# ChicyChen/LOCO-Edit

Hardware: AMD Instinct MI355X
Metric: edit-directions/sec (top-5 PMP-Jacobian SVD @256^2) + vT cos-sim vs ref (higher is better)
Workload: dtype bf16x3 (split-bf16 MFMA operands, fp32 accumulate + fp32 storage); 1 GPU; CelebA-HQ DDPM 256x256 top-5 local basis (l_eye-sized mask, L=2400), t=0.6T, 12 power iterations, one GPU; multi_gpu_form=single, probes_total=5, probes_per_gpu=5, kept=5, n_iter=12, mask_L=2400, weights=synthetic seed 0, streams=2

## Files before the change

### include/loco_hip_diag.h

```cpp
#ifndef LOCO_HIP_DIAG_H
#define LOCO_HIP_DIAG_H
#include "loco_hip.h"
#ifdef __cplusplus
extern "C" {
#endif

int  loco_bench_conv(loco_ctx* ctx, int32_t cin, int32_t cout, int32_t H, int32_t W, int32_t B, int32_t mode,
                     int32_t taps, int32_t tile, int32_t iters, float* ms_avg, void* stream);

typedef struct loco_conv_desc {
    int32_t struct_size;
    int32_t Cin, Cout, Hin, Win, B, taps;
    int32_t stride, upsample, zins, mode, cpg;
    int32_t transposed, accumulate, in_arena, pad;
    int32_t Cin2, cot_cpg;
    float   res_scale;
    int32_t st_cpg;
    const float *weight, *bias;
    const float *in, *bias2, *res;
    const float *prim, *sc, *sh, *mr, *gamma, *tst, *tc;
    const float *in2, *w2, *bias2nd;
    const float *cot_d, *cot_prim, *cot_sc, *cot_sh, *cot_mr, *cot_tc;
    float* out;
    const float *st_prim, *st_mr;
    float* st_out;
    int32_t pool2;
    int32_t st_kind, st_keep;
    float   st_eps;
    int32_t st_keep_cap;
    const float *st_gamma, *st_beta, *st_ss_scale, *st_ss_shift;
    const float *st_sc, *st_sh;
    float *st_o_mr, *st_o_sc, *st_o_sh;
    float *st_o_tst, *st_o_tc;
    float *st_keep_out;
} loco_conv_desc;
int  loco_debug_conv(loco_ctx* ctx, const loco_conv_desc* desc, char* plan, int64_t cap, void* stream);

typedef struct loco_attn_desc {
    int32_t struct_size;
    int32_t kind, pass;
    int32_t T, NH, CH, B;
    int32_t Lt, L, pair, no_workspace;
    const float *q, *k, *v;
    const float *kt, *vt;
    float *P, *o;
    const float *dq, *dk, *dv;
    float* out;
    const float* go;
    float *gq, *gk, *gv;
} loco_attn_desc;
int  loco_debug_attn(loco_ctx* ctx, const loco_attn_desc* desc, char* route, int64_t cap, void* stream);

typedef struct loco_norm_desc {
    int32_t struct_size;
    int32_t op, kind, act, B, C, HW, G, C1, ntA, ntB, accumulate;
    float   eps, base_scale;
    int64_t x_bs, d_bs, base_bs, out_bs, pbs_c, pbs_g, o_bs, t_bs;
// ... 12 lines not shown
```

### loco-edit_amd/csrc/conv.hip

```cpp
#include "kernels.h"

namespace loco {

typedef float f32x16 __attribute__((ext_vector_type(16)));

constexpr int BK = 8;

template <int MODE>
__device__ __forceinline__ float prologue(float d, float x, float sc, float sh, float gamma, float mean,
                                          float rstd, float m1, float m2, int act) {
    if constexpr (MODE == CM_NONE) {
        return d;
    } else if constexpr (MODE == CM_GN_SILU) {
        return act_fwd(fmaf(sc, d, sh), act);
    } else if constexpr (MODE == CM_GN) {
        return fmaf(sc, d, sh);
    } else {
        float xh = (x - mean) * rstd;
        float ds = act_der(fmaf(sc, x, sh), act);
        if constexpr (MODE == CM_TAN_SILU) {
            return ds * sc * (d - m1 - xh * m2);
        } else {
            return rstd * (gamma * ds * d - m1 - xh * m2);
        }
// ... 283 lines not shown
        const int co = (int)(rem / out_plane);
        f32x4_r v = {0.f, 0.f, 0.f, 0.f};
        const float* pp = a.partial + i;
        int s = 0;
        for (; s + 4 <= a.nsplit; s += 4) {
            const f32x4_r p0 = *reinterpret_cast<const f32x4_r*>(pp + (long)s * total);
            const f32x4_r p1 = *reinterpret_cast<const f32x4_r*>(pp + (long)(s + 1) * total);
            const f32x4_r p2 = *reinterpret_cast<const f32x4_r*>(pp + (long)(s + 2) * total);
            const f32x4_r p3 = *reinterpret_cast<const f32x4_r*>(pp + (long)(s + 3) * total);
            v += (p0 + p1) + (p2 + p3);
        }
        for (; s < a.nsplit; ++s) v += *reinterpret_cast<const f32x4_r*>(pp + (long)s * total);
        float add = 0.f;
        if (a.bias) add += a.bias[co];
        if (a.bias2) add += a.bias2[(long)b * a.bias2_bs + co];
        v += add;
        if (a.res) v += a.res_scale * *reinterpret_cast<const f32x4_r*>(a.res + (long)b * a.res_bs + rem);
        float* o = a.out + (long)b * a.out_bs + rem;
        if (a.accumulate) v += *reinterpret_cast<const f32x4_r*>(o);
        *reinterpret_cast<f32x4_r*>(o) = v;
    }
}

void launch_conv_splitk_reduce(const ConvArgs& a, hipStream_t st) {
    if (a.nsplit > 1) {
        long total = (long)a.B * a.Cout * a.Hout * a.Wout;
        const bool vec = ((a.Hout * a.Wout) % 4) == 0 && (a.out_bs % 4) == 0 && (a.res_bs % 4) == 0 &&
                         (reinterpret_cast<uintptr_t>(a.out) % 16) == 0 && (reinterpret_cast<uintptr_t>(a.res) % 16) == 0;
        if (vec) {
            int blocks = (int)((total / 4 + 255) / 256);
            if (blocks > 2048) blocks = 2048;
            hipLaunchKernelGGL(conv_splitk_reduce4, dim3(blocks), dim3(256), 0, st, a, total);
            return;
        }
        int blocks = (int)((total + 255) / 256);
        if (blocks > 2048) blocks = 2048;
        hipLaunchKernelGGL(conv_splitk_reduce, dim3(blocks), dim3(256), 0, st, a, total);
    }
}

}
```

### loco-edit_amd/csrc/conv_bf16.hip

```cpp
#include "kernels.h"
#include <cstdio>
#include <cstdlib>

namespace loco {

enum : int { PR_BF16X3 = 0, PR_F16 = 1 };
template <int PR, int TAPS, int MODE> void launch_tile_b(const ConvArgs& a, hipStream_t st);
template <int PR, int MODE> void launch_kcat_b(const ConvArgs& a, hipStream_t st);
template <int PR, int MODE> void launch_pair_b(const ConvArgs& a, hipStream_t st);
void launch_conv_gemm(const ConvArgs& a, hipStream_t st);
template <int PR> void launch_poly_b(const ConvArgs& a, hipStream_t st);
template <int PR> void launch_poly_in_b(const ConvArgs& a, hipStream_t st);

template <int PR>
static void launch_lowp(const ConvArgs& a, int taps, hipStream_t st) {
#ifdef LOCO_DIAG
    if (a.cot_d && (taps != 1 || a.gemm || a.nsplit > 1 || a.Cin2 > 0 || (a.Cout % conv_bf16_tile_couts(a)) != 0 || a.st_kind == ST_TAN || a.st_kind == ST_COT)) {
        fprintf(stderr, "loco: ConvArgs::cot_d on a launch whose epilogue has no norm-cotangent term (taps %d, gemm %d, nsplit %d, Cout %d, st_kind %d)\n",
                taps, a.gemm, a.nsplit, a.Cout, a.st_kind);
        abort();
    }
#endif
    if constexpr (PR == PR_BF16X3) {
        if (taps == 1 && a.gemm) { launch_conv_gemm(a, st); return; }
    }
    if (taps == 9 && a.poly == 2) { launch_poly_in_b<PR>(a, st); return; }
    if (taps == 9 && a.poly) { launch_poly_b<PR>(a, st); return; }
    if (taps == 9 && a.Cin2 > 0) {
        if (a.mode == CM_GN_SILU) launch_kcat_b<PR, CM_GN_SILU>(a, st);
        else if (a.mode == CM_GN_GELU) launch_kcat_b<PR, CM_GN_GELU>(a, st);
        else launch_kcat_b<PR, CM_TAN_SILU>(a, st);
        return;
    }
    if constexpr (PR == PR_BF16X3) {
        if (taps == 9 && a.pair) {
            switch (a.mode) {
                case CM_NONE: launch_pair_b<PR, CM_NONE>(a, st); break;
                case CM_GN_SILU: launch_pair_b<PR, CM_GN_SILU>(a, st); break;
                case CM_TAN_SILU: launch_pair_b<PR, CM_TAN_SILU>(a, st); break;
                default: launch_pair_b<PR, CM_COT_SILU>(a, st); break;
            }
            return;
        }
    }
    if (taps == 9) {
        switch (a.mode) {
            case CM_NONE: launch_tile_b<PR, 9, CM_NONE>(a, st); break;
            case CM_GN_SILU: launch_tile_b<PR, 9, CM_GN_SILU>(a, st); break;
            case CM_GN_GELU: launch_tile_b<PR, 9, CM_GN_GELU>(a, st); break;
            case CM_TAN_SILU: launch_tile_b<PR, 9, CM_TAN_SILU>(a, st); break;
            case CM_COT_SILU: launch_tile_b<PR, 9, CM_COT_SILU>(a, st); break;
            default: launch_tile_b<PR, 9, CM_GN>(a, st); break;
        }
    } else {
// ... 11 lines not shown
```

### loco-edit_amd/csrc/conv_bf16_inst_f.hip

```cpp
#include "conv_bf16_kernel.h"

namespace loco {
template void launch_kcat_b<PR_BF16X3, CM_GN_SILU>(const ConvArgs&, hipStream_t);
template void launch_kcat_b<PR_BF16X3, CM_TAN_SILU>(const ConvArgs&, hipStream_t);
template void launch_kcat_b<PR_BF16X3, CM_GN_GELU>(const ConvArgs&, hipStream_t);
}
```

### loco-edit_amd/csrc/conv_bf16_inst_f_f16.hip

```cpp
#include "conv_bf16_kernel.h"

namespace loco {
template void launch_kcat_b<PR_F16, CM_GN_SILU>(const ConvArgs&, hipStream_t);
template void launch_kcat_b<PR_F16, CM_TAN_SILU>(const ConvArgs&, hipStream_t);
template void launch_kcat_b<PR_F16, CM_GN_GELU>(const ConvArgs&, hipStream_t);
}
```

### loco-edit_amd/csrc/conv_bf16_kernel.h

```cpp
#pragma once
#include "kernels.h"
#include <cstdlib>
#include <type_traits>

namespace loco {


typedef float f32x16 __attribute__((ext_vector_type(16)));
typedef float f32x4 __attribute__((ext_vector_type(4)));
typedef f32x4 f32x4_u __attribute__((aligned(4)));
typedef float f32x2 __attribute__((ext_vector_type(2)));
typedef f32x2 f32x2_u __attribute__((aligned(4)));
typedef __bf16 bf16x8 __attribute__((ext_vector_type(8)));
typedef _Float16 f16x8 __attribute__((ext_vector_type(8)));
typedef short s16x8 __attribute__((ext_vector_type(8)));

enum : int { PR_BF16X3 = 0, PR_F16 = 1 };

constexpr int BKC = 16;
constexpr bool LIVE_MASK = true;
constexpr bool EARLY_W = true;
constexpr int NDUMMY = 8;

__device__ __forceinline__ float sigmoidf2_(float y) { return __builtin_amdgcn_rcpf(1.0f + __expf(-y)); }
// ... 1304 lines not shown
            (void)hipFuncSetAttribute(reinterpret_cast<const void*>(kern), hipFuncAttributeMaxDynamicSharedMemorySize,
                                      160 * 1024);
        }
    }
    hipLaunchKernelGGL(kern, grid, dim3(WM * WN * 64), lds, st, a);
}

template <int PR, int TAPS, int WM, int WN, int TM, int TN, int MODE>
static void launch_one_b(const ConvArgs& a, hipStream_t st) {
    const bool general = a.stride != 1 || a.upsample || a.zins || (a.Cin % BKC) != 0 || !a.in_padded;
    if constexpr (MODE == CM_NONE) {
        if (a.stride == 2) launch_one_b2<PR, TAPS, WM, WN, TM, TN, MODE, 2>(a, st);
        else if (TAPS == 9 && !general) launch_one_b2<PR, TAPS, WM, WN, TM, TN, MODE, 0>(a, st);
        else launch_one_b2<PR, TAPS, WM, WN, TM, TN, MODE, 1>(a, st);
        return;
    }
    if constexpr (MODE == CM_GN_SILU || MODE == CM_TAN_SILU || MODE == CM_GN_GELU) {
        if (general) { launch_one_b2<PR, TAPS, WM, WN, TM, TN, MODE, 1>(a, st); return; }
    }
    launch_one_b2<PR, TAPS, WM, WN, TM, TN, MODE, 0>(a, st);
}


template <int PR, int MODE>
void launch_kcat_b(const ConvArgs& a, hipStream_t st) {
    constexpr int WM = 2, WN = 4, TM = 2, TN = 2, MT = 128, NT = 256;
    const int TW = a.Wout < 32 ? a.Wout : 32, TH = NT / TW;
    size_t lds = (size_t)3 * 3 * MT * rec_bytes<PR>() + 2 * ((size_t)(TW + 2) * (TH + 2) + NDUMMY) * halo_pitch<PR>();
    dim3 grid(((a.Hout * a.Wout) / NT) * ((a.Cout + MT - 1) / MT) * a.B * a.nsplit);
    void (*kern)(ConvArgs);
    if constexpr (PR == PR_F16) kern = &conv_kcat_f16<WM, WN, TM, TN, MODE>;
    else kern = &conv_kcat_bf16x3<WM, WN, TM, TN, MODE>;
    static DeviceOnce once;
    if (first_on_device(once))
        (void)hipFuncSetAttribute(reinterpret_cast<const void*>(kern), hipFuncAttributeMaxDynamicSharedMemorySize, 160 * 1024);
    hipLaunchKernelGGL(kern, grid, dim3(WM * WN * 64), lds, st, a);
}

template <int PR>
void launch_poly_b(const ConvArgs& a, hipStream_t st) {
    ConvArgs v = a;
    v.Cout = 4 * a.Cout; v.Hout = a.Hin; v.Wout = a.Win;
    v.upsample = 0; v.zins = 0; v.stride = 1; v.pad = 1; v.nsplit = 1;
    launch_one_b2<PR, 4, 2, 4, 2, 2, CM_NONE, 0>(v, st);
}

template <int PR>
void launch_poly_in_b(const ConvArgs& a, hipStream_t st) {
    ConvArgs v = a;
    v.Cin = 4 * a.Cin; v.Hin = a.Hin / 2; v.Win = a.Win / 2;
    v.upsample = 0; v.zins = 0; v.stride = 1; v.pad = 1; v.nsplit = 1;
// ... 19 lines not shown
```

### loco-edit_amd/csrc/conv_plan.hip

```cpp
#include "kernels.h"
#include <cstdio>
#include <cstdlib>

namespace loco {

constexpr int BKC = 16;
constexpr int BKF = 8;

static const int kMT[6] = {128, 128, 32, 64, 128, 128}, kNT[6] = {128, 64, 128, 64, 256, 256};

static int env_int(const char* name, int dflt) {
    const char* e = getenv(name);
    return e ? atoi(e) : dflt;
}
static int pick_tile(int Cout, int HW) {
    if (HW >= 128) return Cout > 32 ? 0 : 2;
    return Cout > 64 ? 1 : 3;
}

static int conv_pick_nsplit(int Cin, int Cout, int Hout, int Wout, int B) {
    const int t = pick_tile(Cout, Hout * Wout);
    long blocks = (long)((Hout * Wout) / kNT[t]) * ((Cout + kMT[t] - 1) / kMT[t]) * B;
    int nchunks = (Cin + BKF - 1) / BKF;
    if (blocks >= 384 || nchunks < 8) return 1;
// ... 50 lines not shown
static int conv_bf16_pick_nsplit(int Cin, int Cout, int Hout, int Wout, int B, int chip_share, int taps, int lanes) {
    const int HW = Hout * Wout;
    int t = conv_bf16_pick_tile(Cout, HW, B, -1);
    if (t == 4) t = 5;
    if (taps == 1 && t == 5 && B >= 2 && HW <= kTile0MaxHW) t = 0;
    long blocks = (long)(HW / kNT[t]) * ((Cout + kMT[t] - 1) / kMT[t]) * B;
    int nchunks = (Cin + BKC - 1) / BKC;
    int target = chip_share > 1 ? 256 / chip_share : (lanes == 2 ? 240 : 256);
    if (target < 32) target = 32;
    if (blocks >= target / 2 || nchunks < 8) return 1;
    int want = (int)(target / blocks);
    int maxs = nchunks / 4;
    if (want > maxs) want = maxs;
    if (want > 32) want = 32;
    return want < 1 ? 1 : want;
}

static bool conv_lowp_can_kcat(const ConvArgs& a) {
    static const bool on = env_int("LOCO_KCAT", 1) != 0;
    return on && a.Cin2 > 0 && a.nsplit == 1 && bf16_tile_of(a) == 5 && a.stride == 1 && !a.upsample && !a.zins && a.pad == 1 &&
           (a.Cin % BKC) == 0 && (a.Cin2 % BKC) == 0 && a.in_padded &&
           (a.mode == CM_GN_SILU || a.mode == CM_GN_GELU || a.mode == CM_TAN_SILU);
}
static bool conv_lowp_can_fuse_stats(const ConvArgs& a) {
    return a.nsplit <= 1 && !a.gemm && (a.Cout % conv_bf16_tile_couts(a)) == 0;
}

static bool conv_pair_ok(const ConvArgs& a) {
    static const bool on = env_int("LOCO_CONV_PAIR", 1) != 0;
    if (!on || a.poly || a.Hout * a.Wout < 16384 || a.taps != 9 || a.Cin2 > 0 || a.nsplit != 1 || a.stride != 1 || a.upsample || a.zins ||
        a.pad != 1 || !a.in_padded || (a.Cin % (2 * BKC)) != 0 || (a.Cout % 128) != 0 || (a.Wout % 32) != 0 || (a.Hout % 8) != 0)
        return false;
    if (!(a.mode == CM_NONE || a.mode == CM_GN_SILU || a.mode == CM_TAN_SILU || a.mode == CM_COT_SILU)) return false;
    return a.tile == 5;
}

static ConvArgs conv_shift_batch(const ConvArgs& a, int nb) {
    ConvArgs t = a;
    t.B = a.B - nb;
    t.in += (long)nb * a.in_bs; t.out += (long)nb * a.out_bs;
    if (t.prim) t.prim += (long)nb * a.prim_bs;
    if (t.bias2) t.bias2 += (long)nb * a.bias2_bs;
    if (t.res) t.res += (long)nb * a.res_bs;
    if (t.sc) { t.sc += (long)nb * a.scsh_bs; t.sh += (long)nb * a.scsh_bs; }
    if (t.mr) t.mr += (long)nb * a.mr_bs;
    if (t.tst) t.tst += (long)nb * a.tst_bs;
// ... 94 lines not shown
    ConvLaunch l;
    l.args = x;
    l.s0 = s0;
    l.args.tile = tile_for(x, e.prec, -1);
    l.stats = stats_route(e, q, want, l.args, s0, B, keep_ntile);
    if (l.stats == SR_EPI || l.stats == SR_KEEP) l.ntile = (x.Hout * x.Wout) / conv_bf16_tile_pixels(l.args);
    conv_plan_tile_pair(l.args, e.prec, -1);
    return l;
}

ConvPlan plan_conv(const ConvEnv& e, const ConvArgs& a0, int taps, const StatAsk* q, const ConvArgs* sc) {
    ConvPlan p;
    ConvArgs a = a0;
    a.taps = taps;
    a.gemm = 0;
    a.poly = 0;
    if (a.pool2) {
        if (conv_poly_in_ok(e, a, taps)) a.poly = 2;
        else {
            p.pool_after = true; p.pool_out = a.out; p.pool_out_bs = a.out_bs; p.pool_acc = a.accumulate;
            a.out = a.pool_tmp; a.out_bs = a.pool_tmp_bs; a.Hout = a.Hin; a.Wout = a.Win; a.accumulate = 0; a.pool2 = 0;
        }
    }
    if (sc) {
        ConvArgs t = a;
        t.nsplit = e.prec >= 1 ? conv_bf16_pick_nsplit(a.Cin, a.Cout, a.Hout, a.Wout, a.B, e.chip_share, 9, e.lanes) : 2;
        t.in2 = sc->in; t.in2_bs = sc->in_bs; t.Cin2 = sc->Cin;
        const long per_probe = (long)((a.Hout * a.Wout) / 256) * ((a.Cout + 127) / 128);
        if (e.prec >= 1 && taps == 9 && !short_tail(per_probe, a.B) && !a.bias2 && conv_lowp_can_kcat(t)) {
            a.in2 = sc->in; a.in2_bs = sc->in_bs; a.Cin2 = sc->Cin; a.in2_padded = sc->in_padded;
            a.wb2 = e.prec == 2 ? sc->wh : sc->wb;
            a.bias2 = sc->bias; a.bias2_bs = 0;
            a.res = nullptr;
        } else {
            p.sc_first = true;
            a.res = sc->out; a.res_bs = sc->out_bs;
        }
    }
    if (e.prec == 2) a.wb = a.wh;
    a.no_deep = e.deep1 ? 0 : 1;
    a.nsplit = e.prec >= 1 ? conv_bf16_pick_nsplit(a.Cin, a.Cout, a.Hout, a.Wout, a.B, e.chip_share, taps, e.lanes)
                           : conv_pick_nsplit(a.Cin, a.Cout, a.Hout, a.Wout, a.B);
    if (a.cot_d) {
        ConvArgs t = a;
        t.tile = bf16_tile_of(t);
        const long per_probe = (long)((a.Hout * a.Wout) / conv_bf16_tile_pixels(t)) * ((a.Cout + 127) / 128);
        p.cot = e.prec >= 1 && taps == 1 && a.nsplit == 1 && !short_tail(per_probe, a.B) && conv_lowp_can_fuse_stats(t);
        if (!p.cot) { a.cot_d = nullptr; a.cot_d_bs = 0; a.cot_sx = nullptr; a.cot_tc = nullptr; a.cot_tc_bs = 0; }
    }
    while (a.nsplit > 1 && (size_t)a.nsplit * a.B * a.Cout * a.Hout * a.Wout > e.partial_floats) a.nsplit >>= 1;
    if (a.nsplit < 1) a.nsplit = 1;
    a.partial = e.partial;
    a.partial_floats = e.partial_floats;
    if (!a.poly && conv_poly_ok(e, a, taps)) a.poly = 1;
    if (a.poly == 1) { a.nsplit = 1; a.wb = e.prec == 2 ? a.wph : a.wpb; }
    if (a.poly == 2) { a.nsplit = 1; a.wb = e.prec == 2 ? a.wqh : a.wqb; }
    conv_plan_family(a, e.prec);
    a.tile = tile_for(a, e.prec, -1);
    int split = 1;
    const int tail = e.prec >= 1 && a.nsplit == 1 && a.B >= 2 && !a.gemm && !a.poly ? tail_split(a, e.partial_floats, &split) : 0;
    const bool want = q && q->kind != ST_NONE && e.prec >= 1 && e.fuse_stats;
    if (!tail) {
        p.l[0] = plan_launch(e, q, want, a, 0, a.B, &p.keep_ntile);
        return p;
    }
    const bool per_part = want && q->norm && (q->kind == ST_FWD || (e.fuse_lin && (a.Hout * a.Wout) % 4 == 0));
    p.stats_all = !per_part && q && q->kind != ST_NONE && q->norm;
    const StatAsk* ql = per_part ? q : nullptr;
    const int nb = a.B - tail;
    ConvArgs m = a, t = conv_shift_batch(a, nb);
    m.B = nb;
    t.nsplit = split;
    p.nl = 2;
    p.l[0] = plan_launch(e, ql, want, m, 0, a.B, &p.keep_ntile);
// ... 23 lines not shown

void polyphase_fold_in(int nin, int nout, const float* w, long so, long si, long st, float* out, int noutP) {
    for (int p = 0; p < 2; ++p)
        for (int q = 0; q < 2; ++q)
            for (int i = 0; i < nin; ++i)
                for (int ty = 0; ty < 2; ++ty)
                    for (int tx = 0; tx < 2; ++tx) {
                        const int m = 2 * ty + 1 - p, n = 2 * tx + 1 - q;
                        for (int o = 0; o < nout; ++o) {
                            double acc = 0.0;
                            for (int a = 0; a < 2; ++a)
                                for (int b = 0; b < 2; ++b) {
                                    const int ky = m - a, kx = n - b;
                                    if (ky >= 0 && ky < 3 && kx >= 0 && kx < 3) acc += (double)w[o * so + i * si + (3 * ky + kx) * st];
                                }
                            out[((((long)(2 * p + q) * nin + i) * 4) + 2 * ty + tx) * noutP + o] = (float)acc;
                        }
                    }
}

const char* conv_variant_name(const ConvArgs& a, int taps, int prec) {
    static const char* tiles[6] = {"2,2,2,2", "4,1,1,2", "1,4,1,1", "2,2,1,1", "2,2,2,4", "2,4,2,2"};
    static char names[3][2][6][6][56];
    static char others[3][3][6][40];
    const int mode = (a.mode < 0 || a.mode > 5) ? 2 : a.mode;
    const char* other = nullptr;
    int k = 0, v = mode;
    if (prec && taps == 9 && a.poly) {
        static const char* pn[2][3] = {{"", "conv_mfma_bf16x3<4,2,4,2,2,0>", "conv_mfma_f16<4,2,4,2,2,0>"},
                                       {"", "conv_mfma_bf16x3<4,2,4,2,2,0>+pool", "conv_mfma_f16<4,2,4,2,2,0>+pool"}};
        return pn[a.poly == 2][prec];
    }
    if (prec && taps == 9 && a.Cin2 > 0) other = prec == 1 ? "conv_kcat_bf16x3<2,4,2,2,%d>" : "conv_kcat_f16<2,4,2,2,%d>";
    else if (prec == 1 && taps == 1 && a.gemm) { k = 1; other = "conv_gemm_bf16x3<%d>"; v = a.gemm_tm; }
    else if (prec == 1 && taps == 9 && a.pair) { k = 2; other = "conv_pair_bf16x3<%d>"; }
    if (other) {
        char* n = others[k][prec][v];
        if (!n[0]) snprintf(n, 40, other, v);
        return n;
    }
    int t = a.tile;
    if (t < 0 || t > 5) t = 0;
    int m = mode;
    if (taps != 9 && m != CM_NONE) m = CM_GN;
    if (!prec && m == CM_GN_GELU) m = CM_GN_SILU;
    char* n = names[prec][taps == 9 ? 0 : 1][t][m];
    static const char* kn[3] = {"conv_mfma_f32", "conv_mfma_bf16x3", "conv_mfma_f16"};
    if (!n[0]) snprintf(n, 56, "%s<%d,%s,%d>", kn[prec], taps, tiles[t], m);
    return n;
}

}
```

### loco-edit_amd/csrc/engine.hip

```cpp
#include <hip/hip_runtime.h>

#include <algorithm>
#include <array>
#include <cmath>
#include <cstdio>
#include <cstdlib>
#include <cstring>
#include <map>
#include <memory>
#include <thread>
#include <atomic>
#include <string>
#include <vector>

#include "../../include/loco_hip.h"
#ifdef LOCO_DIAG
#include "../../include/loco_hip_diag.h"
#endif
#include "kernels.h"
#include "program.h"
#ifdef LOCO_DIAG
#include "conv_plan_text.h"
#endif

// ... 58 lines not shown
    float *xK = nullptr, *xV = nullptr;
};

struct HostParam { std::vector<float> data; std::vector<int64_t> shape; bool loaded = false; };

}


struct loco_ctx {
    loco_unet_cfg cfg;
    std::string err;
    std::map<std::string, HostParam> params;
    bool finalized = false;

    std::shared_ptr<const Program> prog;
    std::shared_ptr<Weights> wts;
    std::vector<Tens> tens;
    std::vector<Op> ops;


    float *arenaP = nullptr, *arenaT = nullptr;
    float *statsP = nullptr, *statsT = nullptr;
    double* red = nullptr;
    bool fuse_cot = true;
    float *stpart = nullptr, *stpart2 = nullptr;
    size_t stpart_floats = 0;
    bool fuse_stats = true;
    bool fuse_xattn = true;
    bool deep1 = true;
    bool flash_attn = true;
    float* attn_delta = nullptr;
    float* partial = nullptr;
    size_t partial_floats = 0;
    const float* bench_out = nullptr; int64_t bench_out_count = 0;
#ifdef LOCO_DIAG
    std::string* plan_log = nullptr;
    std::string* attn_log = nullptr;
#endif
    float *tact = nullptr, *tproj = nullptr;
    float* eps_buf = nullptr;
    float* gx0 = nullptr;
    float* ge = nullptr;
    float* tmpA = nullptr;
    double *G = nullptr, *Q = nullptr, *W = nullptr, *gscratch = nullptr;
    double* kry[2] = {nullptr, nullptr};
    int kry_m[2] = {0, 0}, kry_k[2] = {0, 0};
// ... 479 lines not shown
        launch_gn_stats(x, xbs, B, n.C, HW, G, eps_of(c, n), n.gamma, n.beta, s.mr, s.sc, s.sh, SB, c->red, st, rq.ss_scale,
                        rq.ss_shift);
    } else {
        NS sp = nstats(c, c->statsP, n);
        NS stt = nstats(c, rq.stats + (long)s0 * SB, n);
        launch_gn_tstats(x, xbs, rq.prim, 0, B, n.C, HW, G, sp.sc, sp.sh, sp.mr, 0, 0, rq.kind == ST_TAN ? 0 : 1, stt.tst,
                         stt.tc, SB, c->red, st, c->cfg.act);
    }
}

bool run_conv(loco_ctx* c, const ConvArgs& a0, int taps, hipStream_t st, const StatReq* rq = nullptr,
              const ConvArgs* second = nullptr) {
    const size_t span = (size_t)c->cfg.max_batch * c->prog->per_sample;
    auto padded = [&](const float* p) { return (p >= c->arenaP && p < c->arenaP + span) || (p >= c->arenaT && p < c->arenaT + span); };
    ConvArgs a = a0, sc;
    a.act = c->cfg.act;
    if (a.mode == CM_GN_SILU && c->cfg.act == ACT_GELU) a.mode = CM_GN_GELU;
    a.in_padded = padded(a.in);
    if (second) { sc = *second; sc.in_padded = padded(sc.in); }
    ConvEnv e;
    e.prec = c->prec; e.chip_share = c->chip_share; e.lanes = c->lanes_active; e.lane_s0 = c->lane_s0;
    e.partial = c->partial; e.partial_floats = c->partial_floats; e.stpart = c->stpart; e.stpart_floats = c->stpart_floats;
    e.fuse_stats = c->fuse_stats; e.fuse_lin = c->fuse_lin; e.deep1 = c->deep1; e.max_batch = c->cfg.max_batch;
    StatAsk q;
    if (rq) {
        q.kind = rq->kind; q.norm = rq->n != nullptr; q.prim = rq->prim; q.keep = rq->keep; q.keep_floats = rq->keep_floats;
        if (rq->n && rq->n->sx_off >= 0 && c->sxcache) q.sx = c->sxcache + rq->n->sx_off;
    }
    const ConvPlan p = plan_conv(e, a, taps, rq ? &q : nullptr, second ? &sc : nullptr);
    if (p.sc_first) run_conv(c, *second, 1, st);
#ifdef LOCO_DIAG
    if (c->plan_log) conv_plan_text(p, taps, c->prec, *c->plan_log);
#endif
    if (rq && rq->kind != ST_NONE && rq->n) rq->n->ready = true;
    if (rq && rq->keep_ntile) *rq->keep_ntile = p.keep_ntile;
    const int HWo = a.Hout * a.Wout, Gn = c->cfg.gn_groups;
    const long SBs = c->prog->stats_per_sample;
    auto timed = [&](const char* name, double flops, const ConvArgs& y, auto&& launch) {
        loco_ctx::ProfRec r;
        if (c->prof_on) {
            r.name = name; r.flops = flops;
            r.cin = y.Cin; r.cout = y.Cout; r.h = y.Hout; r.b = y.B; r.ns = y.nsplit; r.mode = y.mode; r.taps = taps;
            r.e0 = c->next_event(); r.e1 = c->next_event();
            (void)hipEventRecord(r.e0, st);
        }
        launch();
// ... 989 lines not shown
    }
    return 0;
}

int create_ctx(loco_ctx* c, const loco_unet_cfg* cfg, std::shared_ptr<const Program> prog) {
    c->cfg = *cfg;
    c->prog = std::move(prog);
    const size_t MB = (size_t)cfg->max_batch;
    {
        float *p0 = nullptr, *p1 = nullptr;
        if (dalloc(c, &p0, MB * c->prog->per_sample + 128) || dalloc(c, &p1, MB * c->prog->per_sample + 128)) return -1;
        c->arenaP = p0 + 64; c->arenaT = p1 + 64;
    }
    if (dalloc(c, &c->statsP, MB * c->prog->stats_per_sample) || dalloc(c, &c->statsT, MB * c->prog->stats_per_sample)) return -1;
    if (dalloc(c, &c->red, RED_BYTES) || dalloc(c, &c->red2, RED_BYTES)) return -1;
    if (alloc_state(c)) return -1;
    {
        c->stpart_floats = MB * (size_t)(c->prog->max_tensor / 64 + 1) * 2;
        if (dalloc(c, &c->stpart, c->stpart_floats) || dalloc(c, &c->stpart2, c->stpart_floats)) return -1;
        const char* e = getenv("LOCO_FUSE_STATS");
        c->fuse_stats = !(e && atoi(e) == 0);
        e = getenv("LOCO_FUSE_LIN");
        c->fuse_lin = !(e && atoi(e) == 0);
        e = getenv("LOCO_FUSE_COT");
        c->fuse_cot = !(e && atoi(e) == 0) && cfg->act == ACT_SILU;
        e = getenv("LOCO_DEEP1");
        c->deep1 = !(e && atoi(e) == 0);
        e = getenv("LOCO_FUSE_XATTN");
        c->fuse_xattn = !(e && atoi(e) == 0);
        const char* fa = getenv("LOCO_FLASH_ATTN");
        c->flash_attn = !(fa && atoi(fa) == 0);
        if (dalloc(c, &c->attn_delta, MB * (size_t)c->prog->attn_dmax)) return -1;
    }
    c->partial_floats = (size_t)64 << 20;
    if (dalloc(c, &c->partial, c->partial_floats)) return -1;
    if (dalloc(c, &c->xin_buf, MB * c->prog->n_in) || dalloc(c, &c->t_dev, 4)) return -1;
    if (dalloc(c, &c->eps_buf, MB * c->prog->n_out) || dalloc(c, &c->gx0, MB * c->prog->n_in) || dalloc(c, &c->ge, MB * c->prog->n_out))
        return -1;
    if (dalloc(c, &c->tmpA, (size_t)64 * c->prog->n_in)) return -1;
    if (dalloc(c, &c->G, 64 * 64) || dalloc(c, &c->Q, 64 * 64) || dalloc(c, &c->W, SOLVER_W_GATE + 1)) return -1;
    {
        size_t nblk = ((size_t)c->prog->n_in + 255) / 256;
        if (dalloc(c, &c->gscratch, nblk * 64 * 64 + 4096)) return -1;
    }
    if (dalloc(c, &c->kry[0], KRY_STATE) || dalloc(c, &c->kry[1], KRY_STATE)) return -1;
    if (dalloc(c, &c->alphas, 256) || dalloc(c, &c->cond_add, (size_t)cfg->ch * 4)) return -1;
// ... 933 lines not shown
    float* const keep_buf = small + (small_n - keep_n - (st_req ? up64(2L * d->Cout) : 0));
    if (st_req) {
        srq.kind = ST_TAN; srq.prim = d->st_prim; srq.keep = keep_buf; srq.keep_floats = (size_t)keep_n; srq.keep_ntile = &kept_ntile;
    }
    NormP stn;
    if (st_norm) {
        stn.C = d->Cout; stn.soff = 0; stn.eps = d->st_eps;
        stn.gamma = const_cast<float*>(d->st_gamma); stn.beta = const_cast<float*>(d->st_beta);
        srq.kind = stk; srq.n = &stn; srq.stats = c->statsT;
        srq.ss_scale = d->st_ss_scale; srq.ss_shift = d->st_ss_shift;
        (void)hipMemsetAsync(c->statsT, 0xff, (size_t)B * SBs * sizeof(float), st);
        if (st_lin) {
            NS sp = nstats(c, c->statsP, stn);
            (void)copy(sp.sc, d->st_sc, d->Cout); (void)copy(sp.sh, d->st_sh, d->Cout); (void)copy(sp.mr, d->st_mr, 2L * Gs);
            srq.prim = d->st_prim;
            if (stk == ST_COT) {
                stn.sx_off = sx_st;
                launch_gn_cache(d->st_prim, d->Cout, Hout * Wout, d->Cout / Gs, sp.sc, sp.sh, sp.mr, c->sxcache + sx_st, st, c->cfg.act);
            }
        }
        if (st_kept) { srq.keep = keep_buf; srq.keep_floats = (size_t)keep_n; srq.keep_ntile = &kept_ntile; }
    }
    bool keep_short = false;
    const bool rode = run_conv(c, a, taps, st, (st_req || st_norm) ? &srq : nullptr, d->Cin2 > 0 ? &n2 : nullptr);
    c->plan_log = nullptr;
    c->cfg.act = act0;
    if (st_norm) {
        NS so = nstats(c, c->statsT, stn);
        auto rows = [&](float* dst, const float* src, long w) {
            return hipMemcpy2DAsync(dst, (size_t)w * sizeof(float), src, (size_t)SBs * sizeof(float), (size_t)w * sizeof(float), (size_t)B,
                                    hipMemcpyDeviceToDevice, st);
        };
        if (stk == ST_FWD) { (void)rows(d->st_o_mr, so.mr, 2L * Gs); (void)rows(d->st_o_sc, so.sc, d->Cout); (void)rows(d->st_o_sh, so.sh, d->Cout); }
        else { (void)rows(d->st_o_tst, so.tst, 2L * Gs); (void)rows(d->st_o_tc, so.tc, 2L * d->Cout); }
        if (st_kept && kept_ntile > 0) {
            const long n = (long)B * d->Cout * kept_ntile * 2;
            if (n <= d->st_keep_cap) (void)copy(d->st_keep_out, keep_buf, n);
            else keep_short = true;
        }
    }
    if (st_req) {
        const int G2 = d->Cout / d->st_cpg;
        float* const zero = keep_buf + keep_n;
        (void)hipMemsetAsync(zero, 0, (size_t)up64(2L * d->Cout) * sizeof(float), st);
        (void)hipMemsetAsync(d->st_out, 0xff, (size_t)B * G2 * 2 * sizeof(float), st);
        if (kept_ntile > 0)
            launch_gn_lin_fused_finalize(ST_TAN, keep_buf, d->Cout, kept_ntile, nullptr, 0, B, d->Cout, Hout * Wout, G2, d->st_mr, d->st_out,
// ... 275 lines not shown
```

### loco-edit_amd/csrc/kernels.h

```cpp
#pragma once
#include <hip/hip_runtime.h>
#include <stdint.h>

namespace loco {

struct DeviceOnce { bool seen[64] = {}; };
inline bool first_on_device(DeviceOnce& f) {
    int d = 0;
    (void)hipGetDevice(&d);
    d &= 63;
    if (f.seen[d]) return false;
    f.seen[d] = true;
    return true;
}


enum ConvMode : int {
    CM_NONE = 0,
    CM_GN_SILU = 1,
    CM_GN = 2,
    CM_TAN_SILU = 3,
    CM_COT_SILU = 4,
    CM_GN_GELU = 5,
};
// ... 53 lines not shown
    int poly;
    int pool2; float* pool_tmp; long pool_tmp_bs;
    const void* wqb; const void* wqh;
};

enum PolyKind : int { POLY_UP = 0, POLY_ZINS_PAD2 = 1, POLY_ZINS_PAD1 = 2 };
inline int polyphase_vcout(int C, int a, int b, int co) { return ((a * (C / 64) + co / 64) * 2 + b) * 64 + (co % 64); }
void polyphase_fold(int kind, int nin, int nout, const float* w, long so, long si, long st, float* out);
void polyphase_fold_in(int nin, int nout, const float* w, long so, long si, long st, float* out, int noutP);

void launch_conv(const ConvArgs& a, int taps, hipStream_t st);
void launch_conv_bf16x3(const ConvArgs& a, int taps, hipStream_t st);
void launch_conv_f16(const ConvArgs& a, int taps, hipStream_t st);
void launch_conv_splitk_reduce(const ConvArgs& a, hipStream_t st);

struct ConvEnv {
    int prec = 1;
    int chip_share = 1;
    int lanes = 1, lane_s0 = 0;
    float* partial = nullptr; size_t partial_floats = 0;
    float* stpart = nullptr; size_t stpart_floats = 0;
    bool fuse_stats = true, fuse_lin = true, deep1 = true;
    int max_batch = 1;
};

struct StatAsk {
    int kind = ST_NONE;
    bool norm = false;
    const float2* sx = nullptr;
    const float* prim = nullptr;
    float* keep = nullptr; size_t keep_floats = 0;
};

enum StatRoute : int {
    SR_NONE = 0,
    SR_EPI = 1,
    SR_SPLITK = 2,
    SR_ALONE = 3,
    SR_KEEP = 4,
};

struct ConvLaunch {
    ConvArgs args;
    int s0 = 0;
    int stats = SR_NONE;
    int ntile = 0;
// ... 198 lines not shown
```

### loco-edit_amd/hip.py

```python
from __future__ import annotations

import ctypes as C
import os
from typing import Dict, Optional

import numpy as np
import torch

from .config import UNetConfig

_LIB_PATH = os.environ.get("LOCO_HIP_LIB") or os.path.join(os.path.dirname(os.path.abspath(__file__)), "libloco_hip.so")
_lib = None

DIAG_SYMBOLS = ["loco_bench_conv", "loco_debug_conv", "loco_debug_attn", "loco_debug_norm", "loco_debug_tensor"]

SYMBOLS = [
    "loco_version", "loco_device_count", "loco_create", "loco_fork", "loco_destroy", "loco_last_error",
    "loco_load_param", "loco_params_missing", "loco_unet_forward", "loco_ddim_step", "loco_sched_step",
    "loco_pmp_primal", "loco_pmp_set_second_mask", "loco_pmp_jvp", "loco_pmp_vjp", "loco_orthonormalize", "loco_qr_rows",
    "loco_convergence", "loco_convergence_rows", "loco_krylov_extend", "loco_krylov_ritz", "loco_krylov_left", "loco_null_project", "loco_edit_axpy", "loco_mask_gather", "loco_mask_count",
    "loco_unet_flops", "loco_workspace_bytes", "loco_clock_stamp", "loco_set_side_stream", "loco_timer_start", "loco_timer_stop",
    "loco_profile_enable", "loco_profile_report", "loco_set_precision", "loco_get_precision", "loco_set_streams", "loco_set_chip_share",
    "loco_set_cond", "loco_set_context", "loco_lincomb", "loco_masked_axpby", "loco_latent_sample",
    "loco_text_create", "loco_text_load_param", "loco_text_params_missing", "loco_text_encode", "loco_text_last_error",
# ... 18 lines not shown
        ("num_levels", C.c_int32), ("ch_mult", C.c_int32 * 8), ("num_res_blocks", C.c_int32),
        ("num_attn_res", C.c_int32), ("attn_resolutions", C.c_int32 * 8), ("gn_groups", C.c_int32),
        ("gn_eps", C.c_float), ("max_batch", C.c_int32),
        ("arch", C.c_int32), ("num_head_channels", C.c_int32), ("learn_sigma", C.c_int32),
        ("context_dim", C.c_int32), ("context_len", C.c_int32),
        ("scale_shift_norm", C.c_int32), ("resblock_updown", C.c_int32), ("num_heads", C.c_int32),
        ("transformer_depth", C.c_int32),
        ("act", C.c_int32), ("res_scale", C.c_float), ("added_kv", C.c_int32),
        ("time_cond_proj_dim", C.c_int32),
    ]


class LocoConvDesc(C.Structure):
    _PTRS = ("weight", "bias", "in", "bias2", "res", "prim", "sc", "sh", "mr", "gamma", "tst", "tc", "in2", "w2", "bias2nd",
             "cot_d", "cot_prim", "cot_sc", "cot_sh", "cot_mr", "cot_tc", "out", "st_prim", "st_mr", "st_out")
    _ST_PTRS = ("st_gamma", "st_beta", "st_ss_scale", "st_ss_shift", "st_sc", "st_sh", "st_o_mr", "st_o_sc", "st_o_sh", "st_o_tst",
                "st_o_tc", "st_keep_out")
    _HOST = ("weight", "bias", "w2", "bias2nd")
    _fields_ = ([("struct_size", C.c_int32)] +
                [(k, C.c_int32) for k in ("Cin", "Cout", "Hin", "Win", "B", "taps", "stride", "upsample", "zins", "mode", "cpg",
                                          "transposed", "accumulate", "in_arena", "pad", "Cin2", "cot_cpg")] +
                [("res_scale", C.c_float), ("st_cpg", C.c_int32)] + [(k, C.c_void_p) for k in _PTRS] + [("pool2", C.c_int32)] +
                [("st_kind", C.c_int32), ("st_keep", C.c_int32), ("st_eps", C.c_float), ("st_keep_cap", C.c_int32)] +
                [(k, C.c_void_p) for k in _ST_PTRS])
    _PTRS = _PTRS + _ST_PTRS


class LocoNormDesc(C.Structure):
    OPS = {"gn_stats": 0, "gn_tstats": 1, "gn_apply": 2, "gn_cache": 3, "gn_fused_finalize": 4, "gn_fused_finalize_cat": 5,
           "gn_lin_fused_finalize": 6, "ctx_groupnorm": 7}
    _PTRS = ("x", "d", "base", "gamma", "beta", "ss_scale", "ss_shift", "sc", "sh", "mr", "tst", "partA", "partB",
             "o_mr", "o_sc", "o_sh", "o_tst", "o_tc", "out")
    _fields_ = ([("struct_size", C.c_int32)] +
                [(k, C.c_int32) for k in ("op", "kind", "act", "B", "C", "HW", "G", "C1", "ntA", "ntB", "accumulate")] +
                [("eps", C.c_float), ("base_scale", C.c_float)] +
                [(k, C.c_int64) for k in ("x_bs", "d_bs", "base_bs", "out_bs", "pbs_c", "pbs_g", "o_bs", "t_bs")] +
                [(k, C.c_void_p) for k in _PTRS])


class LocoAttnDesc(C.Structure):
    _PTRS = ("q", "k", "v", "kt", "vt", "P", "o", "dq", "dk", "dv", "out", "go", "gq", "gk", "gv")
    _fields_ = ([("struct_size", C.c_int32)] +
                [(k, C.c_int32) for k in ("kind", "pass_", "T", "NH", "CH", "B", "Lt", "L", "pair", "no_workspace")] +
                [(k, C.c_void_p) for k in _PTRS])


class LocoTextCfg(C.Structure):
# ... 1063 lines not shown
```

Baseline: 20.27 edit-directions/s.

## Allow K-concatenated shortcut convs and norm-cotangent epilogue under split-K

Residual-block shortcut 1x1 convs can now be folded into the main 3x3 conv through K-concatenation even when the conv runs with split-K. A smaller 4,1,1,2 kcat tile variant is added, and nsplit is trimmed so no split ends up empty. The norm-cotangent term for 1x1 convs, previously only fused when nsplit was 1, is now applied inside a new vectorized split-K reduce kernel. Both paths aim to remove separate shortcut conv launches and extra elementwise passes over activations, at the cost of more template instantiations and more planner complexity.

```diff
diff --git a/include/loco_hip_diag.h b/include/loco_hip_diag.h
--- a/include/loco_hip_diag.h
+++ b/include/loco_hip_diag.h
@@ -33,6 +33,7 @@
     float *st_o_mr, *st_o_sc, *st_o_sh;
     float *st_o_tst, *st_o_tc;
     float *st_keep_out;
+    int32_t kcat_split;
 } loco_conv_desc;
 int  loco_debug_conv(loco_ctx* ctx, const loco_conv_desc* desc, char* plan, int64_t cap, void* stream);
 
diff --git a/loco-edit_amd/csrc/conv.hip b/loco-edit_amd/csrc/conv.hip
--- a/loco-edit_amd/csrc/conv.hip
+++ b/loco-edit_amd/csrc/conv.hip
@@ -329,11 +329,54 @@
     }
 }
 
+__global__ __launch_bounds__(256) void conv_splitk_reduce4_cot(ConvArgs a, long total) {
+    const long out_plane = (long)a.Hout * a.Wout;
+    const long per_b = (long)a.Cout * out_plane;
+    for (long i = ((long)blockIdx.x * blockDim.x + threadIdx.x) * 4; i < total; i += (long)gridDim.x * blockDim.x * 4) {
+        const int b = (int)(i / per_b);
+        const long rem = i - (long)b * per_b;
+        const int co = (int)(rem / out_plane);
+        const f32x4_r d = *reinterpret_cast<const f32x4_r*>(a.cot_d + (long)b * a.cot_d_bs + rem);
+        const f32x4_r* sp4 = reinterpret_cast<const f32x4_r*>(a.cot_sx + rem);
+        const f32x4_r r0 = sp4[0], r1 = sp4[1];
+        const float* tcp = a.cot_tc + (long)b * a.cot_tc_bs + 2 * co;
+        const float c1 = tcp[0], c2 = tcp[1];
+        f32x4_r v = {0.f, 0.f, 0.f, 0.f};
+        const float* pp = a.partial + i;
+        int s = 0;
+        for (; s + 4 <= a.nsplit; s += 4) {
+            const f32x4_r p0 = *reinterpret_cast<const f32x4_r*>(pp + (long)s * total);
+            const f32x4_r p1 = *reinterpret_cast<const f32x4_r*>(pp + (long)(s + 1) * total);
+            const f32x4_r p2 = *reinterpret_cast<const f32x4_r*>(pp + (long)(s + 2) * total);
+            const f32x4_r p3 = *reinterpret_cast<const f32x4_r*>(pp + (long)(s + 3) * total);
+            v += (p0 + p1) + (p2 + p3);
+        }
+        for (; s < a.nsplit; ++s) v += *reinterpret_cast<const f32x4_r*>(pp + (long)s * total);
+        float* o = a.out + (long)b * a.out_bs + rem;
+        if (a.accumulate) v += *reinterpret_cast<const f32x4_r*>(o);
+        v[0] += fmaf(r0[0], d[0], -fmaf(r0[1], c2, c1));
+        v[1] += fmaf(r0[2], d[1], -fmaf(r0[3], c2, c1));
+        v[2] += fmaf(r1[0], d[2], -fmaf(r1[1], c2, c1));
+        v[3] += fmaf(r1[2], d[3], -fmaf(r1[3], c2, c1));
+        float add = 0.f;
+        if (a.bias) add += a.bias[co];
+        if (a.bias2) add += a.bias2[(long)b * a.bias2_bs + co];
+        v += add;
+        *reinterpret_cast<f32x4_r*>(o) = v;
+    }
+}
+
 void launch_conv_splitk_reduce(const ConvArgs& a, hipStream_t st) {
     if (a.nsplit > 1) {
         long total = (long)a.B * a.Cout * a.Hout * a.Wout;
         const bool vec = ((a.Hout * a.Wout) % 4) == 0 && (a.out_bs % 4) == 0 && (a.res_bs % 4) == 0 &&
                          (reinterpret_cast<uintptr_t>(a.out) % 16) == 0 && (reinterpret_cast<uintptr_t>(a.res) % 16) == 0;
+        if (a.cot_d) {
+            int blocks = (int)((total / 4 + 255) / 256);
+            if (blocks > 2048) blocks = 2048;
+            hipLaunchKernelGGL(conv_splitk_reduce4_cot, dim3(blocks), dim3(256), 0, st, a, total);
+            return;
+        }
         if (vec) {
             int blocks = (int)((total / 4 + 255) / 256);
             if (blocks > 2048) blocks = 2048;
diff --git a/loco-edit_amd/csrc/conv_bf16.hip b/loco-edit_amd/csrc/conv_bf16.hip
--- a/loco-edit_amd/csrc/conv_bf16.hip
+++ b/loco-edit_amd/csrc/conv_bf16.hip
@@ -6,7 +6,11 @@
 
 enum : int { PR_BF16X3 = 0, PR_F16 = 1 };
 template <int PR, int TAPS, int MODE> void launch_tile_b(const ConvArgs& a, hipStream_t st);
-template <int PR, int MODE> void launch_kcat_b(const ConvArgs& a, hipStream_t st);
+template <int PR, int MODE, int WM, int WN, int TM, int TN> void launch_kcat_b(const ConvArgs& a, hipStream_t st);
+template <int PR, int MODE> static void launch_kcat_tile(const ConvArgs& a, hipStream_t st) {
+    if (a.tile == 1) launch_kcat_b<PR, MODE, 4, 1, 1, 2>(a, st);
+    else launch_kcat_b<PR, MODE, 2, 4, 2, 2>(a, st);
+}
 template <int PR, int MODE> void launch_pair_b(const ConvArgs& a, hipStream_t st);
 void launch_conv_gemm(const ConvArgs& a, hipStream_t st);
 template <int PR> void launch_poly_b(const ConvArgs& a, hipStream_t st);
@@ -15,7 +19,7 @@
 template <int PR>
 static void launch_lowp(const ConvArgs& a, int taps, hipStream_t st) {
 #ifdef LOCO_DIAG
-    if (a.cot_d && (taps != 1 || a.gemm || a.nsplit > 1 || a.Cin2 > 0 || (a.Cout % conv_bf16_tile_couts(a)) != 0 || a.st_kind == ST_TAN || a.st_kind == ST_COT)) {
+    if (a.cot_d && (taps != 1 || a.gemm || a.Cin2 > 0 || (a.Cout % conv_bf16_tile_couts(a)) != 0 || a.st_kind == ST_TAN || a.st_kind == ST_COT)) {
         fprintf(stderr, "loco: ConvArgs::cot_d on a launch whose epilogue has no norm-cotangent term (taps %d, gemm %d, nsplit %d, Cout %d, st_kind %d)\n",
                 taps, a.gemm, a.nsplit, a.Cout, a.st_kind);
         abort();
@@ -27,9 +31,9 @@
     if (taps == 9 && a.poly == 2) { launch_poly_in_b<PR>(a, st); return; }
     if (taps == 9 && a.poly) { launch_poly_b<PR>(a, st); return; }
     if (taps == 9 && a.Cin2 > 0) {
-        if (a.mode == CM_GN_SILU) launch_kcat_b<PR, CM_GN_SILU>(a, st);
-        else if (a.mode == CM_GN_GELU) launch_kcat_b<PR, CM_GN_GELU>(a, st);
-        else launch_kcat_b<PR, CM_TAN_SILU>(a, st);
+        if (a.mode == CM_GN_SILU) launch_kcat_tile<PR, CM_GN_SILU>(a, st);
+        else if (a.mode == CM_GN_GELU) launch_kcat_tile<PR, CM_GN_GELU>(a, st);
+        else launch_kcat_tile<PR, CM_TAN_SILU>(a, st);
         return;
     }
     if constexpr (PR == PR_BF16X3) {
diff --git a/loco-edit_amd/csrc/conv_bf16_inst_f.hip b/loco-edit_amd/csrc/conv_bf16_inst_f.hip
--- a/loco-edit_amd/csrc/conv_bf16_inst_f.hip
+++ b/loco-edit_amd/csrc/conv_bf16_inst_f.hip
@@ -1,7 +1,7 @@
 #include "conv_bf16_kernel.h"
 
 namespace loco {
-template void launch_kcat_b<PR_BF16X3, CM_GN_SILU>(const ConvArgs&, hipStream_t);
-template void launch_kcat_b<PR_BF16X3, CM_TAN_SILU>(const ConvArgs&, hipStream_t);
-template void launch_kcat_b<PR_BF16X3, CM_GN_GELU>(const ConvArgs&, hipStream_t);
+template void launch_kcat_b<PR_BF16X3, CM_GN_SILU, 2, 4, 2, 2>(const ConvArgs&, hipStream_t);
+template void launch_kcat_b<PR_BF16X3, CM_TAN_SILU, 2, 4, 2, 2>(const ConvArgs&, hipStream_t);
+template void launch_kcat_b<PR_BF16X3, CM_GN_GELU, 2, 4, 2, 2>(const ConvArgs&, hipStream_t);
 }
diff --git a/loco-edit_amd/csrc/conv_bf16_inst_f_f16.hip b/loco-edit_amd/csrc/conv_bf16_inst_f_f16.hip
--- a/loco-edit_amd/csrc/conv_bf16_inst_f_f16.hip
+++ b/loco-edit_amd/csrc/conv_bf16_inst_f_f16.hip
@@ -1,7 +1,7 @@
 #include "conv_bf16_kernel.h"
 
 namespace loco {
-template void launch_kcat_b<PR_F16, CM_GN_SILU>(const ConvArgs&, hipStream_t);
-template void launch_kcat_b<PR_F16, CM_TAN_SILU>(const ConvArgs&, hipStream_t);
-template void launch_kcat_b<PR_F16, CM_GN_GELU>(const ConvArgs&, hipStream_t);
+template void launch_kcat_b<PR_F16, CM_GN_SILU, 2, 4, 2, 2>(const ConvArgs&, hipStream_t);
+template void launch_kcat_b<PR_F16, CM_TAN_SILU, 2, 4, 2, 2>(const ConvArgs&, hipStream_t);
+template void launch_kcat_b<PR_F16, CM_GN_GELU, 2, 4, 2, 2>(const ConvArgs&, hipStream_t);
 }
diff --git a/loco-edit_amd/csrc/conv_bf16_inst_h.hip b/loco-edit_amd/csrc/conv_bf16_inst_h.hip
--- /dev/null
+++ b/loco-edit_amd/csrc/conv_bf16_inst_h.hip
@@ -0,0 +1,10 @@
+#include "conv_bf16_kernel.h"
+
+namespace loco {
+template void launch_kcat_b<PR_BF16X3, CM_GN_SILU, 4, 1, 1, 2>(const ConvArgs&, hipStream_t);
+template void launch_kcat_b<PR_BF16X3, CM_TAN_SILU, 4, 1, 1, 2>(const ConvArgs&, hipStream_t);
+template void launch_kcat_b<PR_BF16X3, CM_GN_GELU, 4, 1, 1, 2>(const ConvArgs&, hipStream_t);
+template void launch_kcat_b<PR_F16, CM_GN_SILU, 4, 1, 1, 2>(const ConvArgs&, hipStream_t);
+template void launch_kcat_b<PR_F16, CM_TAN_SILU, 4, 1, 1, 2>(const ConvArgs&, hipStream_t);
+template void launch_kcat_b<PR_F16, CM_GN_GELU, 4, 1, 1, 2>(const ConvArgs&, hipStream_t);
+}
diff --git a/loco-edit_amd/csrc/conv_bf16_kernel.h b/loco-edit_amd/csrc/conv_bf16_kernel.h
--- a/loco-edit_amd/csrc/conv_bf16_kernel.h
+++ b/loco-edit_amd/csrc/conv_bf16_kernel.h
@@ -1350,11 +1350,14 @@
 }
 
 
-template <int PR, int MODE>
+template <int PR, int MODE, int WM, int WN, int TM, int TN>
 void launch_kcat_b(const ConvArgs& a, hipStream_t st) {
-    constexpr int WM = 2, WN = 4, TM = 2, TN = 2, MT = 128, NT = 256;
+    constexpr int MT = WM * TM * 32, NT = WN * TN * 32;
+    static_assert(MT == 128, "K-concatenated launches: 128-cout tiles");
     const int TW = a.Wout < 32 ? a.Wout : 32, TH = NT / TW;
     size_t lds = (size_t)3 * 3 * MT * rec_bytes<PR>() + 2 * ((size_t)(TW + 2) * (TH + 2) + NDUMMY) * halo_pitch<PR>();
+    const size_t stage_bytes = (size_t)WM * 32 * NT * 4;
+    if (lds < stage_bytes) lds = stage_bytes;
     dim3 grid(((a.Hout * a.Wout) / NT) * ((a.Cout + MT - 1) / MT) * a.B * a.nsplit);
     void (*kern)(ConvArgs);
     if constexpr (PR == PR_F16) kern = &conv_kcat_f16<WM, WN, TM, TN, MODE>;
diff --git a/loco-edit_amd/csrc/conv_plan.hip b/loco-edit_amd/csrc/conv_plan.hip
--- a/loco-edit_amd/csrc/conv_plan.hip
+++ b/loco-edit_amd/csrc/conv_plan.hip
@@ -96,6 +96,13 @@
            (a.Cin % BKC) == 0 && (a.Cin2 % BKC) == 0 && a.in_padded &&
            (a.mode == CM_GN_SILU || a.mode == CM_GN_GELU || a.mode == CM_TAN_SILU);
 }
+static bool conv_lowp_can_kcat_split(const ConvArgs& a) {
+    static const bool on = env_int("LOCO_KCAT", 1) != 0;
+    const int tile = bf16_tile_of(a);
+    return on && a.Cin2 > 0 && a.nsplit > 1 && (tile == 5 || tile == 1) && ((a.Hout * a.Wout) % kNT[tile]) == 0 && a.stride == 1 &&
+           !a.upsample && !a.zins && a.pad == 1 && (a.Cin % BKC) == 0 && (a.Cin2 % BKC) == 0 && a.in_padded &&
+           (a.mode == CM_GN_SILU || a.mode == CM_GN_GELU || a.mode == CM_TAN_SILU);
+}
 static bool conv_lowp_can_fuse_stats(const ConvArgs& a) {
     return a.nsplit <= 1 && !a.gemm && (a.Cout % conv_bf16_tile_couts(a)) == 0;
 }
@@ -236,12 +243,20 @@
             a.out = a.pool_tmp; a.out_bs = a.pool_tmp_bs; a.Hout = a.Hin; a.Wout = a.Win; a.accumulate = 0; a.pool2 = 0;
         }
     }
+    auto ws_nsplit = [&](int ns) {
+        while (ns > 1 && (size_t)ns * a.B * a.Cout * a.Hout * a.Wout > e.partial_floats) ns >>= 1;
+        return ns < 1 ? 1 : ns;
+    };
+    bool kcat_split = false;
     if (sc) {
         ConvArgs t = a;
         t.nsplit = e.prec >= 1 ? conv_bf16_pick_nsplit(a.Cin, a.Cout, a.Hout, a.Wout, a.B, e.chip_share, 9, e.lanes) : 2;
         t.in2 = sc->in; t.in2_bs = sc->in_bs; t.Cin2 = sc->Cin;
         const long per_probe = (long)((a.Hout * a.Wout) / 256) * ((a.Cout + 127) / 128);
-        if (e.prec >= 1 && taps == 9 && !short_tail(per_probe, a.B) && !a.bias2 && conv_lowp_can_kcat(t)) {
+        const bool kcat1 = e.prec >= 1 && taps == 9 && !short_tail(per_probe, a.B) && !a.bias2 && conv_lowp_can_kcat(t);
+        kcat_split = !kcat1 && e.kcat_split && e.prec >= 1 && taps == 9 && !a.bias2 && !a.pool2 && ws_nsplit(t.nsplit) > 1 &&
+                     conv_lowp_can_kcat_split(t);
+        if (kcat1 || kcat_split) {
             a.in2 = sc->in; a.in2_bs = sc->in_bs; a.Cin2 = sc->Cin; a.in2_padded = sc->in_padded;
             a.wb2 = e.prec == 2 ? sc->wh : sc->wb;
             a.bias2 = sc->bias; a.bias2_bs = 0;
@@ -260,10 +275,25 @@
         t.tile = bf16_tile_of(t);
         const long per_probe = (long)((a.Hout * a.Wout) / conv_bf16_tile_pixels(t)) * ((a.Cout + 127) / 128);
         p.cot = e.prec >= 1 && taps == 1 && a.nsplit == 1 && !short_tail(per_probe, a.B) && conv_lowp_can_fuse_stats(t);
+        static const bool split_cot = env_int("LOCO_KCAT_SPLIT_COT", 1) != 0;
+        if (!p.cot && split_cot && e.kcat_split && e.prec >= 1 && taps == 1 && ws_nsplit(a.nsplit) > 1 && !short_tail(per_probe, a.B) &&
+            (!q || q->kind == ST_NONE)) {
+            ConvArgs u = t;
+            u.nsplit = 1;
+            auto al16 = [](const void* ptr) { return (reinterpret_cast<uintptr_t>(ptr) % 16) == 0; };
+            p.cot = conv_lowp_can_fuse_stats(u) && !a.res && ((a.Hout * a.Wout) % 4) == 0 && (a.out_bs % 4) == 0 &&
+                    (a.cot_d_bs % 4) == 0 && al16(a.out) && al16(a.cot_d) && al16(a.cot_sx);
+        }
         if (!p.cot) { a.cot_d = nullptr; a.cot_d_bs = 0; a.cot_sx = nullptr; a.cot_tc = nullptr; a.cot_tc_bs = 0; }
     }
     while (a.nsplit > 1 && (size_t)a.nsplit * a.B * a.Cout * a.Hout * a.Wout > e.partial_floats) a.nsplit >>= 1;
     if (a.nsplit < 1) a.nsplit = 1;
+    if (kcat_split) {
+        const int n1 = a.Cin / BKC, n2 = a.Cin2 / BKC, nmax = n1 > n2 ? n1 : n2;
+        if (a.nsplit > nmax) a.nsplit = nmax;
+        auto last_empty = [](int n, int s) { return (long)(s - 1) * ((n + s - 1) / s) >= n; };
+        while (a.nsplit > 1 && last_empty(n1, a.nsplit) && last_empty(n2, a.nsplit)) --a.nsplit;
+    }
     a.partial = e.partial;
     a.partial_floats = e.partial_floats;
     if (!a.poly && conv_poly_ok(e, a, taps)) a.poly = 1;
@@ -333,7 +363,7 @@
 const char* conv_variant_name(const ConvArgs& a, int taps, int prec) {
     static const char* tiles[6] = {"2,2,2,2", "4,1,1,2", "1,4,1,1", "2,2,1,1", "2,2,2,4", "2,4,2,2"};
     static char names[3][2][6][6][56];
-    static char others[3][3][6][40];
+    static char others[4][3][6][40];
     const int mode = (a.mode < 0 || a.mode > 5) ? 2 : a.mode;
     const char* other = nullptr;
     int k = 0, v = mode;
@@ -342,7 +372,8 @@
                                        {"", "conv_mfma_bf16x3<4,2,4,2,2,0>+pool", "conv_mfma_f16<4,2,4,2,2,0>+pool"}};
         return pn[a.poly == 2][prec];
     }
-    if (prec && taps == 9 && a.Cin2 > 0) other = prec == 1 ? "conv_kcat_bf16x3<2,4,2,2,%d>" : "conv_kcat_f16<2,4,2,2,%d>";
+    if (prec && taps == 9 && a.Cin2 > 0 && a.tile == 1) { k = 3; other = prec == 1 ? "conv_kcat_bf16x3<4,1,1,2,%d>" : "conv_kcat_f16<4,1,1,2,%d>"; }
+    else if (prec && taps == 9 && a.Cin2 > 0) other = prec == 1 ? "conv_kcat_bf16x3<2,4,2,2,%d>" : "conv_kcat_f16<2,4,2,2,%d>";
     else if (prec == 1 && taps == 1 && a.gemm) { k = 1; other = "conv_gemm_bf16x3<%d>"; v = a.gemm_tm; }
     else if (prec == 1 && taps == 9 && a.pair) { k = 2; other = "conv_pair_bf16x3<%d>"; }
     if (other) {
diff --git a/loco-edit_amd/csrc/engine.hip b/loco-edit_amd/csrc/engine.hip
--- a/loco-edit_amd/csrc/engine.hip
+++ b/loco-edit_amd/csrc/engine.hip
@@ -104,6 +104,7 @@
     float *arenaP = nullptr, *arenaT = nullptr;
     float *statsP = nullptr, *statsT = nullptr;
     double* red = nullptr;
+    bool kcat_split = true;
     bool fuse_cot = true;
     float *stpart = nullptr, *stpart2 = nullptr;
     size_t stpart_floats = 0;
@@ -629,6 +630,7 @@
     e.prec = c->prec; e.chip_share = c->chip_share; e.lanes = c->lanes_active; e.lane_s0 = c->lane_s0;
     e.partial = c->partial; e.partial_floats = c->partial_floats; e.stpart = c->stpart; e.stpart_floats = c->stpart_floats;
     e.fuse_stats = c->fuse_stats; e.fuse_lin = c->fuse_lin; e.deep1 = c->deep1; e.max_batch = c->cfg.max_batch;
+    e.kcat_split = c->kcat_split;
     StatAsk q;
     if (rq) {
         q.kind = rq->kind; q.norm = rq->n != nullptr; q.prim = rq->prim; q.keep = rq->keep; q.keep_floats = rq->keep_floats;
@@ -1664,6 +1666,8 @@
         c->fuse_stats = !(e && atoi(e) == 0);
         e = getenv("LOCO_FUSE_LIN");
         c->fuse_lin = !(e && atoi(e) == 0);
+        e = getenv("LOCO_KCAT_SPLIT");
+        c->kcat_split = !(e && atoi(e) == 0);
         e = getenv("LOCO_FUSE_COT");
         c->fuse_cot = !(e && atoi(e) == 0) && cfg->act == ACT_SILU;
         e = getenv("LOCO_DEEP1");
@@ -2643,7 +2647,10 @@
         if (st_kept) { srq.keep = keep_buf; srq.keep_floats = (size_t)keep_n; srq.keep_ntile = &kept_ntile; }
     }
     bool keep_short = false;
+    const bool kcat_split_ctx = c->kcat_split;
+    c->kcat_split = d->kcat_split != 0;
     const bool rode = run_conv(c, a, taps, st, (st_req || st_norm) ? &srq : nullptr, d->Cin2 > 0 ? &n2 : nullptr);
+    c->kcat_split = kcat_split_ctx;
     c->plan_log = nullptr;
     c->cfg.act = act0;
     if (st_norm) {
diff --git a/loco-edit_amd/csrc/kernels.h b/loco-edit_amd/csrc/kernels.h
--- a/loco-edit_amd/csrc/kernels.h
+++ b/loco-edit_amd/csrc/kernels.h
@@ -99,6 +99,7 @@
     float* stpart = nullptr; size_t stpart_floats = 0;
     bool fuse_stats = true, fuse_lin = true, deep1 = true;
     int max_batch = 1;
+    bool kcat_split = false;
 };
 
 struct StatAsk {
diff --git a/loco-edit_amd/hip.py b/loco-edit_amd/hip.py
--- a/loco-edit_amd/hip.py
+++ b/loco-edit_amd/hip.py
@@ -64,7 +64,7 @@
                                           "transposed", "accumulate", "in_arena", "pad", "Cin2", "cot_cpg")] +
                 [("res_scale", C.c_float), ("st_cpg", C.c_int32)] + [(k, C.c_void_p) for k in _PTRS] + [("pool2", C.c_int32)] +
                 [("st_kind", C.c_int32), ("st_keep", C.c_int32), ("st_eps", C.c_float), ("st_keep_cap", C.c_int32)] +
-                [(k, C.c_void_p) for k in _ST_PTRS])
+                [(k, C.c_void_p) for k in _ST_PTRS] + [("kcat_split", C.c_int32)])
     _PTRS = _PTRS + _ST_PTRS
 
 
```

Measured after the change: 20.46 edit-directions/s, median of 6. About the same (+1.0%).
